# JacobPorter/FastNeighborNet

Measured on AMD Instinct MI355X. Metric: sec to circular order, n=32768 taxa (+ achieved HBM GB/s), lower is better.
Workload: dtype f64

## Files before the change

fastneighbornet_amd/csrc/fnn_hip.hip:

```cpp
#include <hip/hip_runtime.h>

#include <dlfcn.h>

#include <cmath>
#include <new>

#include "fnn_chain.h"
#include "fnn_engine.h"

namespace fnn {

struct fnn_nccl_id { char internal[FNN_COMM_ID_BYTES]; };

constexpr int SCAN_TW = 512;
constexpr int SCAN_TH = 32;
constexpr int SCAN_THREADS = 256;

static_assert(sizeof(Cand) == 24, "rec_publish / rec_fetch move a Cand as three 8-byte words");
__device__ inline uint64_t rec_check_word(const Cand& c, uint32_t tag) {
    return __builtin_bit_cast(uint64_t, c.q) ^ (c.key * 0x9E3779B97F4A7C15ULL) ^
           ((uint64_t)(uint32_t)c.si | ((uint64_t)(uint32_t)c.sj << 32)) ^ (((uint64_t)tag + 1ULL) * 0xBF58476D1CE4E5B9ULL);
}
__device__ inline void rec_publish(Cand* p, const Cand& c, uint64_t* chk, uint32_t tag) {
    __hip_atomic_store(chk, rec_check_word(c, tag), __ATOMIC_RELAXED, __HIP_MEMORY_SCOPE_AGENT);
    uint64_t* w = (uint64_t*)p;
    __hip_atomic_store(w + 0, __builtin_bit_cast(uint64_t, c.q), __ATOMIC_RELAXED, __HIP_MEMORY_SCOPE_AGENT);
    __hip_atomic_store(w + 1, c.key, __ATOMIC_RELAXED, __HIP_MEMORY_SCOPE_AGENT);
    __hip_atomic_store(w + 2, (uint64_t)(uint32_t)c.si | ((uint64_t)(uint32_t)c.sj << 32), __ATOMIC_RELAXED, __HIP_MEMORY_SCOPE_AGENT);
}
__device__ inline Cand rec_fetch(const Cand* p) {
    uint64_t* w = (uint64_t*)p;
    const uint64_t a = __hip_atomic_load(w + 0, __ATOMIC_RELAXED, __HIP_MEMORY_SCOPE_AGENT);
    const uint64_t b = __hip_atomic_load(w + 1, __ATOMIC_RELAXED, __HIP_MEMORY_SCOPE_AGENT);
    const uint64_t x = __hip_atomic_load(w + 2, __ATOMIC_RELAXED, __HIP_MEMORY_SCOPE_AGENT);
    Cand c;
    c.q = __builtin_bit_cast(double, a);
    c.key = b;
// ... 665 lines not shown
    if (!d.st->done) {
        for (int i = threadIdx.x; i < nrecs; i += 1024) {
            Cand c = src[i];
            if (cand_better(c, best)) best = c;
        }
    }
    return block_reduce<16>(best, sh);
}

__global__ __launch_bounds__(1024) void k_reduce_local(Dev d, int nrecs) {
    __shared__ Cand sh[16];
    Cand best = reduce_records(d, d.recs, nrecs, sh);
    if (threadIdx.x == 0) d.gsend[0] = best;
}


template <int EPT>
struct ChainLds {
    double wtot[CH_T / 64];
    double s;
    int slot_count;
    int32_t E[CH_T];
    int32_t flags[CH_T];
    int32_t slot[CH_T];
    uint64_t own[CH_T], sc[CH_T];
    double vals[CH_NSLOT][EPT];
    double spv[CH_T];
    ChRec prec[CH_NSLOT];
    double pend_A0[CH_NSLOT];
    int32_t pend_cnt[CH_NSLOT];
    uint64_t wk[CH_T / 64];
    int32_t wr[CH_T / 64];
    int32_t fail;
};

__device__ __forceinline__ uint64_t shfl_up_u64(uint64_t v, int d) {
    return (uint64_t)__shfl_up((unsigned long long)v, d, 64);
}
__device__ __forceinline__ int readlane_i32(int v, int lane) { return __builtin_amdgcn_readlane(v, lane); }
__device__ __forceinline__ uint64_t readlane_u64(uint64_t v, int lane) {
    uint32_t lo = (uint32_t)__builtin_amdgcn_readlane((int)(uint32_t)v, lane);
    uint32_t hi = (uint32_t)__builtin_amdgcn_readlane((int)(uint32_t)(v >> 32), lane);
    return ((uint64_t)hi << 32) | lo;
}

__device__ __forceinline__ uint64_t readfirstlane_u64(uint64_t v) {
    uint32_t lo = (uint32_t)__builtin_amdgcn_readfirstlane((int)(uint32_t)v);
    uint32_t hi = (uint32_t)__builtin_amdgcn_readfirstlane((int)(uint32_t)(v >> 32));
    return ((uint64_t)hi << 32) | lo;
}

__device__ __forceinline__ void chain_serial_global(double& s, const double* buf, int start, int cnt, int m) {
    for (int i = 0; i < cnt; i++)
        if (start + i < m) s += buf[chain_addr(start + i)];
}

__device__ int g_chain_form = 2;
__device__ int g_chain_stop_after = 0;

template <int EPT, int MODE = 0>
__device__ __forceinline__ double block_chain_sum(const double* __restrict__ buf, int m, int guard_bits, ChainLds<EPT>& L,
                                  ChainStats* stats) {
    const int stop_after = stats ? g_chain_stop_after : 0;
    static_assert(EPT % 2 == 0 && EPT <= 64, "EPT");
    const int tid = threadIdx.x, lane = tid & 63, w = tid >> 6;
    ChainStats cs{0, 0, 0, 0};
    if (tid == 0) L.s = 0.0;
    for (int base = 0; base < m; base += CH_T * EPT) {
        double s_in = 0.0;
        if (MODE != 2) {
        if (tid == 0) L.slot_count = 0;
        static_assert(EPT == CH_EPT, "the buffer layout is fixed to CH_EPT addends per thread");
        double a[EPT];
        const int idx0 = base + tid * EPT;
        const double* src = buf + base + 2 * tid;
#pragma unroll
        for (int i = 0; i < EPT; i += 2) {
            double2 v = make_double2(0.0, 0.0);
            if (idx0 + i < m) v = *reinterpret_cast<const double2*>(src + (i >> 1) * (2 * CH_T));
            a[i] = v.x;
            a[i + 1] = (idx0 + i + 1 < m) ? v.y : 0.0;
        }
        double loc = 0.0;
#pragma unroll
        for (int i = 0; i < EPT; i++) loc += a[i];
        double inc = loc;
#pragma unroll
        for (int d = 1; d < 64; d <<= 1) {
            const double t = __shfl_up(inc, d, 64);
            if (lane >= d) inc += t;
        }
// ... 155 lines not shown
        if (!tm) { r.kind = CHR_CONST; r.E0 = E_first; r.c0 = mono_inc_bits(msum(ci, inm)); return r; }
        const int jt = __builtin_ctzll(tm);
        const unsigned long long lo = inm & ((1ULL << jt) - 1ULL), hi = inm & ~((2ULL << jt) - 1ULL);
        r.kind = CHR_SPLIT; r.E0 = E_first; r.E1 = E_first;
        r.c0 = mono_inc_bits(msum(ci, lo)); r.c1 = mono_inc_bits(msum(ci, hi));
        r.sp = __builtin_bit_cast(double, readlane_u64(f2u(al), jt));
        return r;
    }
    const int js = __builtin_ctzll(bad);
    const unsigned long long lo = inm & ((1ULL << js) - 1ULL), hi = inm & ~((2ULL << js) - 1ULL);
    int32_t E1 = -1;
    if (hi) {
        const int jn = __builtin_ctzll(hi);
        E1 = __builtin_amdgcn_readlane(El, jn);
        if (__ballot(((hi >> lane) & 1ULL) && (!okl || El != E1))) return r;
    }
    bool tie0 = false, inv0 = false, tie1 = false, inv1 = false;
    const double c0l = lo ? konst(E_first, tie0, inv0) : 0.0;
    const double c1l = hi ? konst(E1, tie1, inv1) : 0.0;
    if (__ballot((((lo >> lane) & 1ULL) && (tie0 || inv0)) || (((hi >> lane) & 1ULL) && (tie1 || inv1)))) return r;
    r.kind = CHR_SPLIT;
    r.E0 = lo ? E_first : -1; r.c0 = lo ? mono_inc_bits(msum(c0l, lo)) : 0;
    r.E1 = hi ? E1 : -1; r.c1 = hi ? mono_inc_bits(msum(c1l, hi)) : 0;
    r.sp = __builtin_bit_cast(double, readlane_u64(f2u(al), js));
    return r;
}

template <int EPT>
__device__ __attribute__((noinline)) double block_chain_sum_rare(const double* __restrict__ buf, int m, int guard_bits, ChainLds<EPT>* L,
                                                               ChainStats* stats) {
    return block_chain_sum<EPT>(buf, m, guard_bits, *L, stats);
}

template <int EPT>
__device__ __forceinline__ double block_chain_sum2(const double* __restrict__ buf, int m, int guard_bits, ChainLds<EPT>& L,
                                                   ChainStats* stats) {
    static_assert(EPT == CH_EPT, "the buffer layout is fixed to CH_EPT addends per thread");
    const int tid = threadIdx.x, lane = tid & 63, w = tid >> 6;
    ChainStats cs{0, 0, 0, 0};
    if (tid == 0) { L.s = 0.0; L.fail = 0; }
    for (int base = 0; base < m; base += CH_T * EPT) {
        if (tid == 0) L.slot_count = 0;
        double a[EPT];
        const int idx0 = base + tid * EPT;
        const double* src = buf + base + 2 * tid;
#pragma unroll
        for (int i = 0; i < EPT; i += 2) {
            double2 v = make_double2(0.0, 0.0);
            if (idx0 + i < m) v = *reinterpret_cast<const double2*>(src + (i >> 1) * (2 * CH_T));
            a[i] = v.x;
            a[i + 1] = (idx0 + i + 1 < m) ? v.y : 0.0;
        }
        double l4[4] = {0.0, 0.0, 0.0, 0.0};
#pragma unroll
        for (int i = 0; i < EPT; i++) l4[i & 3] += a[i];
        const double loc = (l4[0] + l4[1]) + (l4[2] + l4[3]);
        double inc = loc;
#pragma unroll
        for (int d = 1; d < 64; d <<= 1) {
            const double t = __shfl_up(inc, d, 64);
            if (lane >= d) inc += t;
        }
        if (lane == 63) L.wtot[w] = inc;
        __syncthreads();
        double wpre = 0.0;
        for (int k = 0; k < w; k++) wpre += L.wtot[k];
        const double s_in = L.s;
        const double A0 = s_in + (wpre + (inc - loc));
        const int cnt = idx0 >= m ? 0 : (m - idx0 < EPT ? m - idx0 : EPT);
        ChRec r;
        r.kind = CHR_EMPTY; r.E0 = r.E1 = -1; r.c0 = r.c1 = 0; r.sp = 0.0;
        int slot = -1;
        if (cnt > 0) {
            int32_t E = -1;
            int nt = 0;
            uint64_t c = 0;
            if (chain_predict(A0, A0 + loc, guard_bits != 0, E) && chain_consts(a, 0, cnt, E, c, &nt, nullptr) && nt == 0) {
                r.kind = CHR_CONST; r.E0 = E; r.c0 = c;
            } else {
                r.kind = CHR_SERIAL;
                slot = atomicAdd(&L.slot_count, 1);
                if (slot < CH_NSLOT) {
#pragma unroll
                    for (int i = 0; i < EPT; i++) L.vals[slot][i] = a[i];
                    L.pend_A0[slot] = A0;
                    L.pend_cnt[slot] = cnt;
                } else slot = -1;
            }
        }
        __syncthreads();
        {
            const int ns = L.slot_count < CH_NSLOT ? L.slot_count : CH_NSLOT;
            for (int sl = w; sl < ns; sl += CH_T / 64) {
                const double al = lane < EPT ? L.vals[sl][lane < EPT ? lane : 0] : 0.0;
                const ChRec pr = chain_record_wave(al, L.pend_cnt[sl], L.pend_A0[sl], guard_bits != 0);
                if (lane == 0) L.prec[sl] = pr;
            }
        }
        __syncthreads();
        if (slot >= 0) r = L.prec[slot];
        const int32_t tailE = r.kind == CHR_CONST ? r.E0 : (r.kind == CHR_SPLIT ? r.E1 : -2);
        int32_t prevTail = __shfl_up(tailE, 1, 64);
        L.E[tid] = tailE;
        __syncthreads();
        if (lane == 0) prevTail = tid > 0 ? L.E[tid - 1] : -2;
        const bool ebreak = r.kind == CHR_CONST && prevTail != r.E0;
        int rr = (r.kind == CHR_SPLIT || r.kind == CHR_SERIAL || ebreak) ? 1 : 0;
        uint64_t kk = r.kind == CHR_CONST ? r.c0 : (r.kind == CHR_SPLIT ? (r.E1 >= 0 ? r.c1 : 0) : 0);
        const int r_own = rr;
        const uint64_t k_own = kk;
#pragma unroll
        for (int d = 1; d < 64; d <<= 1) {
            const int pr = __shfl_up(rr, d, 64);
            const uint64_t pk = shfl_up_u64(kk, d);
            if (lane >= d) {
                if (!rr) { const uint64_t t = pk + kk; kk = t > (1ULL << 60) ? (1ULL << 60) : t; }
                rr |= pr;
            }
        }
        if (lane == 63) { L.wr[w] = rr; L.wk[w] = kk; }
        __syncthreads();
        uint64_t X = 0;
        for (int q = 0; q < w; q++) { const uint64_t t = X + L.wk[q]; X = L.wr[q] ? L.wk[q] : (t > (1ULL << 60) ? (1ULL << 60) : t); }
        uint64_t after;
        { const uint64_t t = X + kk; after = rr ? kk : (t > (1ULL << 60) ? (1ULL << 60) : t); }
        uint64_t xin = shfl_up_u64(after, 1);
        if (lane == 0) xin = X;
        (void)r_own; (void)k_own;
        const bool evt = r.kind == CHR_SPLIT || r.kind == CHR_SERIAL || (ebreak && xin != 0);
        __syncthreads();
        L.E[tid] = prevTail;
        L.flags[tid] = r.kind | (evt ? 4 : 0);
        L.slot[tid] = r.kind == CHR_SERIAL ? slot : r.E0;
        L.own[tid] = r.c0;
        L.sc[tid] = xin;
        L.spv[tid] = r.sp;
        const int lastT = ((m - base < CH_T * EPT ? m - base : CH_T * EPT) - 1) / EPT;
        if (tid == lastT) { L.wk[0] = after; L.wr[0] = tailE; }
        __syncthreads();
        if (r.kind == CHR_SERIAL && tid <= lastT) cs.mixed++;
        if (w == 0) {
            uint64_t sb = readfirstlane_u64(f2u(s_in));
            bool ok = true;
            auto apply = [&](int E, uint64_t c) {
                if (c == 0) return;
                if (mono_apply_pattern(sb, E, c, c)) cs.runs++;
                else ok = false;
            };
            for (int ww = 0; ww < CH_T / 64 && ok; ww++) {
                if (ww * 64 > lastT) break;
                const int id = ww * 64 + lane;
                const int rf = L.flags[id], rEin = L.E[id], rs = L.slot[id];
                const uint64_t rc0 = L.own[id], rx = L.sc[id];
                const double rsp = L.spv[id];
                unsigned long long em = __ballot((rf & 4) != 0 && id <= lastT);
                while (em && ok) {
                    const int e = __builtin_ctzll(em);
                    em &= em - 1;
                    const int kind = readlane_i32(rf, e) & 3, Ein = readlane_i32(rEin, e), sl = readlane_i32(rs, e);
                    const uint64_t x = readlane_u64(rx, e), c0 = readlane_u64(rc0, e);
                    if (kind == CHR_CONST) apply(Ein, x);
                    else if (kind == CHR_SPLIT) {
                        const int E0 = sl;
                        if (E0 >= 0 && E0 == Ein) { const uint64_t t = x + c0; apply(E0, t > (1ULL << 60) ? (1ULL << 60) : t); }
                        else { apply(Ein, x); if (E0 >= 0) apply(E0, c0); }
                        if (!ok) break;
                        const double sv = u2f(sb) + u2f(readlane_u64(f2u(rsp), e));
                        sb = readfirstlane_u64(f2u(sv));
                    } else {
                        apply(Ein, x);
                        if (!ok) break;
                        double sv = u2f(sb);
                        if (sl >= 0) {
                            const double* pv = L.vals[sl];
#pragma unroll
                            for (int j = 0; j < EPT; j++) sv += pv[j];
                        } else chain_serial_global(sv, buf, base + (ww * 64 + e) * EPT, EPT, m);
                        sb = readfirstlane_u64(f2u(sv));
                    }
                }
            }
            if (ok) apply((int)L.wr[0], L.wk[0]);
            if (lane == 0) { L.s = u2f(sb); if (!ok) L.fail = 1; }
        }
        __syncthreads();
        if (L.fail) break;
    }
    __syncthreads();
    if (L.fail) {
        ChainStats c1{0, 0, 0, 0};
        const double r1 = block_chain_sum_rare<EPT>(buf, m, guard_bits, &L, stats ? &c1 : nullptr);
        if (stats && tid == 0) { stats->runs = cs.runs + c1.runs; stats->mixed = cs.mixed + c1.mixed; stats->run_fail = 1 + c1.run_fail; stats->thread_fail = c1.thread_fail; }
        return r1;
    }
    if (stats) {
        __shared__ int mixed_total;
        if (tid == 0) mixed_total = 0;
        __syncthreads();
        if (cs.mixed) atomicAdd(&mixed_total, cs.mixed);
        __syncthreads();
        if (tid == 0) { cs.mixed = mixed_total; *stats = cs; }
    }
    return L.s;
}

struct PreSrc { const double *pD, *pSx, *pT; int64_t pld; };
__device__ __forceinline__ void build_targets_wave(State& st, const Dev& d, const PreSrc& src, const int32_t pendU, const int32_t tpU, const double* tfin) {
    const int lane = threadIdx.x & 63;
    const int nops = __builtin_amdgcn_readfirstlane(st.nops);
    const int U = __builtin_amdgcn_readfirstlane(st.U), m = __builtin_amdgcn_readfirstlane(st.m);
    const int ev_finish = __builtin_amdgcn_readfirstlane(st.ev_finish);
    static_assert(sizeof(Op) == 32, "Op is read as 8 dwords");
    const int opw = lane < 8 * MAX_OPS ? reinterpret_cast<const int32_t*>(st.ops)[lane] : 0;
    int err = 0;
    int Sl = -1, nS = 0;
    auto add_slot = [&](int sl) {
        if (__ballot(lane < nS && Sl == sl)) return;
        if (nS >= MAX_S) { err = 5; return; }
        if (lane == nS) Sl = sl;
        nS++;
    };
// ... 764 lines not shown
        return;
    }
    if (st->stall || st->la_hit) {
        if (HELP && threadIdx.x == 0) job_post(d, jobtag, 0u);
        return;
    }
    state_in(S.lst, st);
    if (threadIdx.x == 0) S.tkon = 0;
    Cand best = reduce_records(d, src, st->rl_active ? 1 : nrecs, shc);
    __syncthreads();
    decide_step<HELP, false>(d, S, L, best, jobtag);
    __syncthreads();
    if (threadIdx.x == 0) S.lst.rl_active = 0;
    __syncthreads();
    state_out(st, S.lst);
}

constexpr int TRK_THREADS = 1024;
constexpr int TRK_GROUP = 16;
constexpr int TRK_FLAG = 32 * 65;
constexpr int TRK_BAD = 32 * 67;

__device__ __forceinline__ void chain_workgroup(const Dev& d, ChainLds<CH_EPT>& L) {
    State* st = d.st;
    if (!st->chain_pending) return;
    const int32_t cU = st->chain_U, cm = st->chain_m;
    const unsigned evtag = (unsigned)st->n_events;
    const double usx = block_chain_sum2<CH_EPT>(d.chain, cm, CH_GUARD_BITS, L, nullptr);
    if (threadIdx.x == 0) {
        __hip_atomic_store(reinterpret_cast<uint64_t*>(d.Sx + cU), __builtin_bit_cast(uint64_t, usx), __ATOMIC_RELAXED, __HIP_MEMORY_SCOPE_AGENT);
        __hip_atomic_store(reinterpret_cast<uint64_t*>(d.Sx + cU + 1), __builtin_bit_cast(uint64_t, usx), __ATOMIC_RELAXED, __HIP_MEMORY_SCOPE_AGENT);
        __hip_atomic_store(reinterpret_cast<uint64_t*>(&upre_behind_ticket(d)->usx), __builtin_bit_cast(uint64_t, usx), __ATOMIC_RELAXED, __HIP_MEMORY_SCOPE_AGENT);
        asm volatile("s_waitcnt vmcnt(0)" ::: "memory");
        __threadfence();
        __hip_atomic_store(d.ticket + TRK_FLAG, evtag, __ATOMIC_RELAXED, __HIP_MEMORY_SCOPE_AGENT);
    }
}

__device__ __forceinline__ void sweep_exact_item(const Dev& d, int64_t r, const TrackArgs& ta, Cand& bx) {
    const int32_t half = (ta.m + 1) / 2;
    const int32_t fi = ta.nf0 + (int32_t)(r / half), cp = (int32_t)(r % half);
    if (fi >= ta.nf) return;
    const int32_t f0 = fresh_slot(d, fi, ta.m);
    if (f0 < 0) return;
    const int32_t s2 = 2 * cp;
    if (s2 >= ta.m || s2 == f0) return;
    const double* F0 = d.D + (int64_t)f0 * d.ld + s2;
    const double* F1 = F0 + d.ld;
    const double a0 = F0[0], a1 = F0[1], b0 = F1[0], b1 = F1[1];
    if (f0 > s2)
        scan_micro(f0, s2, ta.m, ta.twoP, ta.cm2, a0, a1, b0, b1, d.Sx[f0], d.Sx[f0 + 1], d.spos[f0], d.spos[f0 + 1],
                   d.Sx[s2], d.Sx[s2 + 1], d.spos[s2], d.spos[s2 + 1], bx);
    else
        scan_micro(s2, f0, ta.m, ta.twoP, ta.cm2, a0, b0, a1, b1, d.Sx[s2], d.Sx[s2 + 1], d.spos[s2], d.spos[s2 + 1],
                   d.Sx[f0], d.Sx[f0 + 1], d.spos[f0], d.spos[f0 + 1], bx);
}

constexpr int TRK_REC_U = 1024;

struct SpecialOut { double val, tu, tv; };
__device__ __forceinline__ SpecialOut special_wave(const Dev& d, const State& lst, double* blk, double* sxl, double* tl, int32_t* berr, double* chain_dst) {
    const int lane = threadIdx.x & 63;
    const int nS = __builtin_amdgcn_readfirstlane(lst.nS);
    const int32_t Sl = lane < nS ? lst.S[lane < MAX_S ? lane : 0] : -1;
    const int m_old = __builtin_amdgcn_readfirstlane(lst.m_old), twoP_old = 2 * __builtin_amdgcn_readfirstlane(lst.P_old);
    const int m = __builtin_amdgcn_readfirstlane(lst.m), twoP = 2 * __builtin_amdgcn_readfirstlane(lst.P);
    const int xs = __builtin_amdgcn_readfirstlane(lst.xs), ys = __builtin_amdgcn_readfirstlane(lst.ys);
// ... 363 lines not shown
                    c = rec_fetch(&d.recs[TRK_REC_U + i]);
                    if (rec_check_word(c, tag) != __hip_atomic_load(d.rchk + TRK_REC_U + i, __ATOMIC_RELAXED, __HIP_MEMORY_SCOPE_AGENT)) stale = true;
                    if (cand_better(c, bu)) bu = c;
                }
            }
            stale = __ballot(stale) != 0ULL;
            if (!stale) break;
            reread = true;
            __threadfence();
        }
        b = wave_reduce(b);
        if (ta.approx) bu = wave_reduce(bu);
        if (threadIdx.x == 0) {
            sh[0] = b;
            shu[0] = bu;
            if (badword != 0u) {
                d.ticket[TRK_BAD] = 0u;
                lastflag = 2;
            }
            if (stale) lastflag = 2;
            if (reread) S.lst.n_ev_persistent++;
        }
    }
    __syncthreads();
    best = sh[0];
    bestu = shu[0];
    if (lastflag == 2) {
        giveup = true;
        if (d.strict && threadIdx.x == 0) S.lst.error = 13;
    }
    __syncthreads();
    TRK_TICK(5);
    if (ta.approx && !giveup) {
        const double dmax = __builtin_bit_cast(double, st->dmax_bits);
        const double margin = 2.0 * eps_u + 192.0 * 1.1102230246251565e-16 * ((double)st->n + 4.0) * dmax + 1e-300;
        const bool certain = (bestu.q - margin > best.q) || (bestu.q == inf_f64());
        if (!certain) {
            if (threadIdx.x == 0) {
                const unsigned want = evtag0;
                const long long t_wait = (long long)wall_clock64();
                while (__hip_atomic_load(d.ticket + TRK_FLAG, __ATOMIC_RELAXED, __HIP_MEMORY_SCOPE_AGENT) != want) {
                    if ((long long)wall_clock64() - t_wait > TRK_WAIT_TICKS) { lst.error = 10; break; }
                    __builtin_amdgcn_s_sleep(2);
                }
                __threadfence();
                lst.n_sweep_waits++;
            }
            __syncthreads();
            Cand bx;
            bx = cand_none();
            for (int64_t r = threadIdx.x; r < items - ta.np; r += TRK_THREADS) sweep_exact_item(d, r, ta, bx);
            bx = block_reduce<TRK_THREADS / 64>(bx, sh);
            if (threadIdx.x == 0) sh[0] = bx;
            __syncthreads();
            bx = sh[0];
            if (cand_better(bx, best)) best = bx;
        }
    }
    if (giveup) { best = cand_none(); }
    if (threadIdx.x == 0) {
        *d.ticket = 0u;
        lst.ev_timed = timed;
        if (giveup) lst.n_sweep_waits++;
        la_track_done(dl, best, ta);
        lst.stall = (!lst.la_hit && !has_scan) ? 1 : 0;
        if (lst.stall) lst.n_stalled++;
    }
    __syncthreads();
// ... 117 lines not shown
__global__ __launch_bounds__(CH_T) void k_chain_flush(Dev d) {
    __shared__ ChainLds<CH_EPT> L;
    chain_workgroup(d, L);
    __syncthreads();
    if (threadIdx.x == 0) d.st->chain_pending = 0;
}

constexpr int SER_CHUNK = 8192;
__device__ __forceinline__ double serial_chain_sum(const double* buf, int m, double* ser) {
    double s = 0.0;
    for (int base = 0; base < m; base += SER_CHUNK) {
        const int cnt = m - base < SER_CHUNK ? m - base : SER_CHUNK;
        for (int i = threadIdx.x; i < cnt; i += CH_T) ser[i] = buf[chain_addr(base + i)];
        __syncthreads();
        if (threadIdx.x == 0) {
#pragma unroll 8
            for (int i = 0; i < cnt; i++) s += ser[i];
        }
        __syncthreads();
    }
    return s;
}

__global__ __launch_bounds__(CH_T) void k_finalize(Dev d) {
    __shared__ ChainLds<CH_EPT> L;
    __shared__ double ser[SER_CHUNK];
    State* st = d.st;
    if (!st->ev_active || st->stall) return;
    double usx = 0.0;
    if (!st->ev_finish) usx = st->nonneg ? block_chain_sum2<CH_EPT>(d.chain, st->m, CH_GUARD_BITS, L, nullptr) : serial_chain_sum(d.chain, st->m, ser);
    if (threadIdx.x == 0) finalize(d, usx);
}

template <int EPT>
__global__ __launch_bounds__(CH_T) void k_test_chain(const double* buf, int m, int guard_bits, double* out, ChainStats* stats) {
    __shared__ ChainLds<EPT> L;
    double r = g_chain_form == 1 ? block_chain_sum<EPT>(buf, m, guard_bits, L, stats) : block_chain_sum2<EPT>(buf, m, guard_bits, L, stats);
    if (threadIdx.x == 0) *out = r;
}

__global__ __launch_bounds__(256) void k_init(Dev d) { init_thread(d, blockIdx.x * 256 + threadIdx.x); }

__global__ __launch_bounds__(256) void k_synth(Dev d, uint64_t seed, int dist) {
    int64_t c = (int64_t)blockIdx.x * 256 + threadIdx.x;
    int64_t r = blockIdx.y;
    if (c >= d.n) return;
    double v = 0.0;
    if (r < c) v = synth_entry(d.n, r, c, seed, dist);
    else if (c < r) v = synth_entry(d.n, c, r, seed, dist);
    d.D[r * d.ld + c] = v;
}

__global__ __launch_bounds__(256) void k_unpack(Dev d, const double* __restrict__ stage, int64_t p0, int32_t row0) {
    const int64_t r = row0 + (int64_t)blockIdx.y;
    const int64_t c = (int64_t)blockIdx.x * 256 + threadIdx.x;
    if (c <= r || c >= d.n) return;
    d.D[r * d.ld + c] = __builtin_nontemporal_load(stage + (packed_row_base(d.n, r) + c - p0));
}

__global__ __launch_bounds__(256) void k_mirror(Dev d) {
    __shared__ double tile[32][33];
    const int bx = blockIdx.x, by = blockIdx.y;
    if (bx < by) return;
    const int tx = threadIdx.x & 31, ty = threadIdx.x >> 5;
    for (int k = ty; k < 32; k += 8) {
        const int64_t r = (int64_t)by * 32 + k, c = (int64_t)bx * 32 + tx;
        tile[k][tx] = (r < d.n && c < d.n && r < c) ? d.D[r * d.ld + c] : 0.0;
    }
    __syncthreads();
    for (int k = ty; k < 32; k += 8) {
// ... 312 lines not shown
        if (!HIPOK(hipMemcpyAsync(&hb, d_bad, sizeof(int), hipMemcpyDeviceToHost, stream)) ||
            !HIPOK(hipStreamSynchronize(stream)))
            return FNN_EHIP;
        *bad = hb;
        return FNN_OK;
    }
    int32_t launch_prep_screen(const Dev& d, int64_t nrows) {
        const int64_t want = (nrows * d.ld + 255) / 256;
        launch(TC_OTHER, false, k_prep_screen, dim3((unsigned)(want < 8192 ? (want > 0 ? want : 1) : 8192)), dim3(256), d, nrows);
        return launched();
    }
    int32_t launch_init(const Dev& d) {
        reset_timing();
        rx_exact_seen = 0; rx_helpers = 0;
        launch(TC_OTHER, false, k_init, grid1(d.n), dim3(256), d);
        return launched();
    }

    dim3 scan_dims(const Dev& d, int32_t m_bound) const {
        int nt = (scan_tile_count(m_bound) + d.world - 1) / d.world;
        return dim3((unsigned)(nt < scan_grid ? (nt > 0 ? nt : 1) : scan_grid));
    }
    bool screen_off = false;
    bool keep_generic_screen() const { return false; }
    bool use_screen(const Dev& d, int32_t m_bound) const { return d.H != nullptr && !screen_off && m_bound >= screen_min_m; }
    int enqueue_scan(const Dev& d, int32_t m_bound, bool sched) {
        const bool screen = use_screen(d, m_bound);
        const bool tscan = timing != 0 && (sched || !screen), tall = timing == 2;
        const bool has_scan = sched || !screen || unsched_scans;
        if (d.la) {
            const bool help = rx_helpers > 0;
            const int fb = (sched || !screen) ? 1 : 0, hs = has_scan ? 1 : 0, tk = ticks ? 1 : 0;
            track_tag = (track_tag % 0x7FFFFFEu) + 1u;
            launch(TC_TRACK, tall, help ? k_track<true> : k_track<false>, dim3(track_grid + 1 + (help ? TRK_NHELP : 0)), dim3(TRK_THREADS),
                   d, fb, fb, hs, track_group, tk, track_tag);
        }
        if (screen && !has_scan) return 0;
        if (screen) {
            static constexpr decltype(&k_screen<true, true>) variants[2][2] = {{k_screen<true, true>, k_screen<false, true>},
                                                                               {k_screen<true, false>, k_screen<false, false>}};
            int nt = (tri_tile_count(m_bound, SCR_TH, SCR_R) + d.world - 1) / d.world;
            const int want = sched ? scan_grid : unsched_grid;
            launch(TC_SCREEN, tscan, variants[!sched][!scan_nt], dim3((unsigned)(nt < want ? (nt > 0 ? nt : 1) : want)), dim3(256), d);
            if (d.la) launch(TC_EMIT, tall, k_emit, dim3(emit_grid), dim3(256), d);
            launch(TC_RESOLVE, tall, k_resolve, dim3(RES_BLOCKS), dim3(1024), d);
            if (tscan) scan_launches++;
            return RES_BLOCKS;
        }
        if (relaxed_min > 0 && m_bound > relaxed_min) {
            int g = relaxed_grid > 0 ? relaxed_grid : (m_bound >= 12288 ? m_bound / 4096 : 1);
            launch(TC_OTHER, tall, k_relaxed, dim3(g > RL_GMAX ? RL_GMAX : g), dim3(RL_T), d, ticks ? 1 : 0);
        }
        const dim3 gs = scan_dims(d, m_bound);
        launch(TC_SCAN, tscan, scan_nt ? k_scan<true> : k_scan<false>, gs, dim3(SCAN_THREADS), d);
        if (tscan) plain_launches++;
        return (int)gs.x;
    }
    void enqueue_rest(const Dev& d, int32_t m_bound, const Cand* src, int nrecs) {
        const bool tall = timing == 2, help = rx_helpers > 0;
        if (nrecs > 0) {
            track_tag = (track_tag % 0x7FFFFFEu) + 1u;
            launch(TC_DECIDE, tall, help ? k_decide<true> : k_decide<false>, dim3(1 + (help ? TRK_NHELP : 0)), dim3(CH_T), d, src, nrecs, track_tag);
        }
        launch(TC_UPDATE, tall, k_update, dim3(grid1(m_bound).x + 1), dim3(256), d, defer_chain ? 1 : 0, ticks ? 1 : 0);
        if (!defer_chain) launch(TC_OTHER, tall, k_finalize, dim3(1), dim3(CH_T), d);
    }
    int32_t launch_event(const Dev& d, int32_t m_bound, bool sched) {
// ... 227 lines not shown
    return FNN_OK;
}
int32_t fnn_comm_init_rccl(fnn_handle* h, int32_t world, int32_t rank, const uint8_t* id, const char* rccl_path) {
    FNN_NEED(h);
    if (!id) return fnn::fail(FNN_EINVAL, "fnn_comm_init_rccl: id is NULL");
    FNN_TRY(
        int32_t rc = h->eng.comm_set(1, world, rank);
        if (rc != FNN_OK) return rc;
        if (h->eng.comm_mode == 0) return FNN_OK;
        rc = h->eng.be.comm_init_rccl(world, rank, id, rccl_path);
        if (rc != FNN_OK) { h->eng.comm_set(0, 1, 0); return fnn::fail(rc, h->eng.be.err()); }
        return FNN_OK;
    )
}
int32_t fnn_comm_init_host(fnn_handle* h, int32_t world, int32_t rank, fnn_allgather_fn fn, void* ctx) {
    FNN_NEED(h);
    if (world > 1 && !fn) return fnn::fail(FNN_EINVAL, "fnn_comm_init_host: callback is NULL");
    FNN_TRY(
        int32_t rc = h->eng.comm_set(2, world, rank);
        if (rc != FNN_OK) return rc;
        h->eng.host_fn = fn;
        h->eng.host_ctx = ctx;
        return FNN_OK;
    )
}

int32_t fnn_test_chain_sum(int32_t device, const double* host_buf, int32_t m, int32_t guard_bits, int32_t ept,
                           double* out, int32_t* stats4) {
    if (!host_buf || m < 0 || !out || ept != fnn::CH_EPT)
        return fnn::fail(FNN_EINVAL, "fnn_test_chain_sum: bad arguments (ept must be 32)");
    hipError_t e;
    if ((e = hipSetDevice(device)) != hipSuccess) return fnn::fail(FNN_EHIP, hipGetErrorString(e));
    const size_t cap = (size_t)fnn::round_up(m > 0 ? m : 1, fnn::CH_SC);
    std::vector<double> perm(cap, 0.0);
    for (int32_t i = 0; i < m; i++) perm[(size_t)fnn::chain_addr(i)] = host_buf[i];
    double* dbuf = nullptr; double* dout = nullptr; fnn::ChainStats* dst = nullptr;
    if (hipMalloc((void**)&dbuf, sizeof(double) * cap) != hipSuccess || hipMalloc((void**)&dout, 8) != hipSuccess ||
        hipMalloc((void**)&dst, sizeof(fnn::ChainStats)) != hipSuccess) {
        (void)hipFree(dbuf); (void)hipFree(dout); (void)hipFree(dst);
        return fnn::fail(FNN_ENOMEM, "fnn_test_chain_sum: hipMalloc failed");
    }
    (void)hipMemcpy(dbuf, perm.data(), sizeof(double) * cap, hipMemcpyHostToDevice);
    {
        int stop = 0;
        if (const char* ev = std::getenv("FNN_CHAIN_STOP")) stop = std::atoi(ev);
        (void)hipMemcpyToSymbol(HIP_SYMBOL(fnn::g_chain_stop_after), &stop, sizeof(int));
        int form = stop ? 1 : 2;
        if (const char* ev = std::getenv("FNN_CHAIN_FORM")) form = std::atoi(ev);
        (void)hipMemcpyToSymbol(HIP_SYMBOL(fnn::g_chain_form), &form, sizeof(int));
    }
    hipLaunchKernelGGL(fnn::k_test_chain<fnn::CH_EPT>, dim3(1), dim3(fnn::CH_T), 0, 0, dbuf, m, guard_bits, dout, dst);
    e = hipDeviceSynchronize();
    if (std::getenv("FNN_CHAIN_TIME")) {
        hipEvent_t e0, e1;
        (void)hipEventCreate(&e0); (void)hipEventCreate(&e1);
        (void)hipEventRecord(e0, 0);
        for (int i = 0; i < 50; i++)
            hipLaunchKernelGGL(fnn::k_test_chain<fnn::CH_EPT>, dim3(1), dim3(fnn::CH_T), 0, 0, dbuf, m, guard_bits, dout, dst);
        (void)hipEventRecord(e1, 0);
        (void)hipEventSynchronize(e1);
        float ms = 0.f;
        (void)hipEventElapsedTime(&ms, e0, e1);
        std::fprintf(stderr, "[fnn] k_test_chain m=%d: %.2f us per launch\n", m, ms * 1e3 / 50);
        (void)hipEventDestroy(e0); (void)hipEventDestroy(e1);
    }
    fnn::ChainStats hs{0, 0, 0, 0};
    if (e == hipSuccess) e = hipMemcpy(out, dout, 8, hipMemcpyDeviceToHost);
    if (e == hipSuccess) e = hipMemcpy(&hs, dst, sizeof(hs), hipMemcpyDeviceToHost);
    (void)hipFree(dbuf); (void)hipFree(dout); (void)hipFree(dst);
    if (e != hipSuccess) return fnn::fail(FNN_EHIP, std::string("fnn_test_chain_sum: ") + hipGetErrorString(e));
    if (stats4) { stats4[0] = hs.runs; stats4[1] = hs.mixed; stats4[2] = hs.run_fail; stats4[3] = hs.thread_fail; }
    return FNN_OK;
}

int32_t fnn_stream_probe(int32_t device, int64_t bytes, int32_t reps, double* gbps_out) {
    if (bytes < (1 << 20) || reps < 1 || !gbps_out) return fnn::fail(FNN_EINVAL, "fnn_stream_probe: bad arguments");
    hipError_t e;
    if ((e = hipSetDevice(device)) != hipSuccess) return fnn::fail(FNN_EHIP, hipGetErrorString(e));
    void* p = nullptr;
    double* sink = nullptr;
    if ((e = hipMalloc(&p, (size_t)bytes)) != hipSuccess) return fnn::fail(FNN_ENOMEM, hipGetErrorString(e));
    if ((e = hipMalloc((void**)&sink, 8)) != hipSuccess) { (void)hipFree(p); return fnn::fail(FNN_ENOMEM, hipGetErrorString(e)); }
    (void)hipMemset(p, 0, (size_t)bytes);
    hipEvent_t e0, e1;
    (void)hipEventCreate(&e0);
    (void)hipEventCreate(&e1);
    int64_t n16 = bytes / 16;
    dim3 g(256 * 8);
    hipLaunchKernelGGL(fnn::k_stream, g, dim3(256), 0, 0, (const double2*)p, n16, sink);
    (void)hipEventRecord(e0, 0);
    for (int i = 0; i < reps; i++) hipLaunchKernelGGL(fnn::k_stream, g, dim3(256), 0, 0, (const double2*)p, n16, sink);
    (void)hipEventRecord(e1, 0);
    e = hipEventSynchronize(e1);
    float ms = 0.f;
    (void)hipEventElapsedTime(&ms, e0, e1);
    (void)hipEventDestroy(e0);
    (void)hipEventDestroy(e1);
    (void)hipFree(p);
    (void)hipFree(sink);
    if (e != hipSuccess || ms <= 0.f) return fnn::fail(FNN_EHIP, "fnn_stream_probe: timing failed");
    *gbps_out = (double)bytes * reps / (ms * 1e-3) / 1e9;
    return FNN_OK;
}

}
```

include/fastnn.h:

```cpp
#ifndef FASTNN_H
#define FASTNN_H

#include <stdint.h>

#ifdef __cplusplus
extern "C" {
#endif

#define FASTNN_ABI_VERSION 2

typedef enum fnn_status {
    FNN_OK      = 0,
    FNN_EINVAL  = -1,
    FNN_ENOMEM  = -2,
    FNN_EHIP    = -3,
    FNN_ERCCL   = -4,
    FNN_ESTATE  = -5,
    FNN_ECAPACITY = -6,
    FNN_EINEXACT = -7
} fnn_status;

enum { FNN_KIND_2WAY = 2, FNN_KIND_3WAY = 3, FNN_KIND_4WAY = 4, FNN_KIND_FINISH = 5 };

typedef struct fnn_opts {
// ... 122 lines not shown
    int64_t outer_iterations;
    int64_t cg_calls;
    int64_t cg_iterations;
    int64_t nsplits;
    double  t_solve_s;
    int64_t reserved[3];
    int32_t route;
    int32_t certified;
    double  kkt_violation;
    double  final_threshold_rel;
    int64_t n_set_aside;
    int64_t capacity;
    int64_t free_set_peak;
    int32_t giveup_reason;
    int32_t pad_;
    int64_t entered, screened_out, departed;
    double  t_alloc_s;
    int64_t reserved2[4];
} fnn_sw_stats;
enum { FNN_SW_ROUTE_CLOSED_FORM = 0, FNN_SW_ROUTE_FROM_BELOW = 1, FNN_SW_ROUTE_REFERENCE = 2 };
enum { FNN_SW_GIVEUP_NONE = 0, FNN_SW_GIVEUP_CAPACITY = 1,
       FNN_SW_GIVEUP_STEPS = 2,
       FNN_SW_GIVEUP_NUMERIC = 3,
       FNN_SW_GIVEUP_DEPARTED = 4,
       FNN_SW_GIVEUP_SETUP = 5 };
int32_t fnn_split_weights_f64(const double* D, int32_t n, int64_t ld, const int32_t* ordering, int32_t device,
                              double* weights_out, fnn_sw_stats* stats);
int32_t fnn_split_weights_sparse_f64(const double* D, int32_t n, int64_t ld, const int32_t* ordering, int32_t device, double threshold,
                                     int64_t* index_out, double* weight_out, int64_t capacity, int64_t* count_out, fnn_sw_stats* stats);
int32_t fnn_split_weights_release_cache(void);

int32_t fnn_test_chain_sum(int32_t device, const double* host_buf, int32_t m, int32_t guard_bits,
                           int32_t ept, double* out, int32_t* stats4);

int32_t fnn_stream_probe(int32_t device, int64_t bytes, int32_t reps, double* gbps_out);

#ifdef __cplusplus
}
#endif
#endif
```

Before: 1.296.

## Rework block chain sum with DPP scans, short-input path, and fewer barriers

Replaces the shuffle-based wave prefix scans in block_chain_sum2 with DPP row/broadcast scans, and replaces the serial cross-wave loops with a wave-level scan. It adds a single-wave serial path for short inputs and skips a barrier when there are no serial slots. The event walk now visits only waves that flagged events. Separately, it drops a __threadfence after s_waitcnt in the update publish, shrinks the track grid to one block in fallback mode, reads margin fields from LDS, and adds tick profiling for the test kernel. These lower barrier and scan latency in the chain-sum hot loop. The dropped fence risks memory-ordering bugs.

```diff
diff --git a/fastneighbornet_amd/csrc/fnn_hip.hip b/fastneighbornet_amd/csrc/fnn_hip.hip
--- a/fastneighbornet_amd/csrc/fnn_hip.hip
+++ b/fastneighbornet_amd/csrc/fnn_hip.hip
@@ -3,6 +3,7 @@
 #include <dlfcn.h>
 
 #include <cmath>
+#include <limits>
 #include <new>
 
 #include "fnn_chain.h"
@@ -734,7 +735,14 @@
     uint64_t wk[CH_T / 64];
     int32_t wr[CH_T / 64];
     int32_t fail;
+    int32_t wtail[CH_T / 64], whead[CH_T / 64];
+    uint64_t emask[CH_T / 64];
+    uint64_t open_k;
+    int32_t open_E;
 };
+constexpr int32_t CH_NOHEAD = INT32_MIN;
+constexpr int CH_SHORT_M = 2048;
+static_assert(CH_SHORT_M <= 64 * CH_EPT, "the short form is one wave: one chunk per lane");
 
 __device__ __forceinline__ uint64_t shfl_up_u64(uint64_t v, int d) {
     return (uint64_t)__shfl_up((unsigned long long)v, d, 64);
@@ -757,8 +765,10 @@
         if (start + i < m) s += buf[chain_addr(start + i)];
 }
 
-__device__ int g_chain_form = 2;
+__device__ int g_chain_form = 0;
 __device__ int g_chain_stop_after = 0;
+constexpr int CH_NTICK = 7;
+__device__ long long g_chain_ticks[CH_NTICK];
 
 template <int EPT, int MODE = 0>
 __device__ __forceinline__ double block_chain_sum(const double* __restrict__ buf, int m, int guard_bits, ChainLds<EPT>& L,
@@ -980,12 +990,84 @@
     return block_chain_sum<EPT>(buf, m, guard_bits, *L, stats);
 }
 
+template <int CTRL, int ROW_MASK>
+__device__ __forceinline__ uint32_t dpp_or0(uint32_t v) {
+    return (uint32_t)__builtin_amdgcn_update_dpp(0, (int)v, CTRL, ROW_MASK, 0xf, false);
+}
+template <int CTRL, int ROW_MASK>
+__device__ __forceinline__ uint64_t dpp_or0_u64(uint64_t v) {
+    const uint32_t lo = dpp_or0<CTRL, ROW_MASK>((uint32_t)v), hi = dpp_or0<CTRL, ROW_MASK>((uint32_t)(v >> 32));
+    return ((uint64_t)hi << 32) | lo;
+}
+__device__ __forceinline__ uint32_t lane_below_u32(uint32_t v) {
+    const uint32_t inrow = dpp_or0<0x111, 0xf>(v), across = dpp_or0<0x142, 0xe>(v);
+    return (threadIdx.x & 15) ? inrow : across;
+}
+__device__ __forceinline__ uint64_t lane_below_u64(uint64_t v) {
+    return ((uint64_t)lane_below_u32((uint32_t)(v >> 32)) << 32) | lane_below_u32((uint32_t)v);
+}
+__device__ __forceinline__ uint64_t sat60(uint64_t t) { return t > (1ULL << 60) ? (1ULL << 60) : t; }
+template <bool ROWS_ONLY>
+__device__ __forceinline__ double scan_add_f64(double x) {
+#define FNN_SCAN_STEP(CTRL, MASK) x += u2f(dpp_or0_u64<CTRL, MASK>(f2u(x)))
+    FNN_SCAN_STEP(0x111, 0xf); FNN_SCAN_STEP(0x112, 0xf); FNN_SCAN_STEP(0x114, 0xf); FNN_SCAN_STEP(0x118, 0xf);
+    if (!ROWS_ONLY) { FNN_SCAN_STEP(0x142, 0xa); FNN_SCAN_STEP(0x143, 0xc); }
+#undef FNN_SCAN_STEP
+    return x;
+}
+template <bool ROWS_ONLY>
+__device__ __forceinline__ void scan_seg(int& rr, uint64_t& kk) {
+#define FNN_SCAN_STEP(CTRL, MASK) do { const int pr = (int)dpp_or0<CTRL, MASK>((uint32_t)rr); const uint64_t pk = dpp_or0_u64<CTRL, MASK>(kk); \
+        if (!rr) kk = sat60(pk + kk); rr |= pr; } while (0)
+    FNN_SCAN_STEP(0x111, 0xf); FNN_SCAN_STEP(0x112, 0xf); FNN_SCAN_STEP(0x114, 0xf); FNN_SCAN_STEP(0x118, 0xf);
+    if (!ROWS_ONLY) { FNN_SCAN_STEP(0x142, 0xa); FNN_SCAN_STEP(0x143, 0xc); }
+#undef FNN_SCAN_STEP
+}
+
 template <int EPT>
+__device__ __forceinline__ double chain_short_sum(const double* __restrict__ buf, int m, ChainLds<EPT>& L) {
+    const int tid = threadIdx.x;
+    if (tid < 64) {
+        double a[EPT];
+        const double* src = buf + 2 * tid;
+#pragma unroll
+        for (int j = 0; j < EPT / 2; j++) {
+            double2 v = make_double2(0.0, 0.0);
+            if (tid * EPT + 2 * j < m) v = *reinterpret_cast<const double2*>(src + j * (2 * CH_T));
+            a[2 * j] = v.x;
+            a[2 * j + 1] = tid * EPT + 2 * j + 1 < m ? v.y : 0.0;
+        }
+        double sv = 0.0;
+        const int nch = (m + EPT - 1) / EPT;
+        for (int t = 0; t < nch; t++) {
+            double s = u2f(readlane_u64(f2u(sv), t > 0 ? t - 1 : 0));
+            if (t == 0) s = 0.0;
+#pragma unroll
+            for (int i = 0; i < EPT; i++) s += a[i];
+            sv = s;
+        }
+        const double res = nch > 0 ? u2f(readlane_u64(f2u(sv), nch > 0 ? nch - 1 : 0)) : 0.0;
+        if (tid == 0) L.s = res;
+    }
+    __syncthreads();
+    return L.s;
+}
+
+template <int EPT, bool PROF = false>
 __device__ __forceinline__ double block_chain_sum2(const double* __restrict__ buf, int m, int guard_bits, ChainLds<EPT>& L,
-                                                   ChainStats* stats) {
+                                                   ChainStats* stats, int short_below = CH_SHORT_M) {
     static_assert(EPT == CH_EPT, "the buffer layout is fixed to CH_EPT addends per thread");
     const int tid = threadIdx.x, lane = tid & 63, w = tid >> 6;
+    const int wu = __builtin_amdgcn_readfirstlane(w);
+    if (m < short_below && m <= 64 * EPT) {
+        if (stats && tid == 0) *stats = ChainStats{0, 0, 0, 0};
+        return chain_short_sum<EPT>(buf, m, L);
+    }
     ChainStats cs{0, 0, 0, 0};
+    const bool prof = PROF && stats != nullptr && tid == 0;
+    long long tk[CH_NTICK] = {0, 0, 0, 0, 0, 0, 0};
+#define CH_TICK(k, dep) do { if (prof) { asm volatile("" :: "v"(dep) : "memory"); tk[k] = (long long)wall_clock64(); } } while (0)
+    CH_TICK(0, tid);
     if (tid == 0) { L.s = 0.0; L.fail = 0; }
     for (int base = 0; base < m; base += CH_T * EPT) {
         if (tid == 0) L.slot_count = 0;
@@ -1003,18 +1085,16 @@
 #pragma unroll
         for (int i = 0; i < EPT; i++) l4[i & 3] += a[i];
         const double loc = (l4[0] + l4[1]) + (l4[2] + l4[3]);
-        double inc = loc;
-#pragma unroll
-        for (int d = 1; d < 64; d <<= 1) {
-            const double t = __shfl_up(inc, d, 64);
-            if (lane >= d) inc += t;
-        }
+        CH_TICK(1, loc);
+        const double inc = scan_add_f64<false>(loc);
         if (lane == 63) L.wtot[w] = inc;
         __syncthreads();
-        double wpre = 0.0;
-        for (int k = 0; k < w; k++) wpre += L.wtot[k];
+        const double wsc = scan_add_f64<true>(lane < CH_T / 64 ? L.wtot[lane & (CH_T / 64 - 1)] : 0.0);
+        const double wbelow = u2f(readlane_u64(f2u(wsc), wu > 0 ? wu - 1 : 0));
+        const double wpre = wu > 0 ? wbelow : 0.0;
         const double s_in = L.s;
         const double A0 = s_in + (wpre + (inc - loc));
+        CH_TICK(2, A0);
         const int cnt = idx0 >= m ? 0 : (m - idx0 < EPT ? m - idx0 : EPT);
         ChRec r;
         r.kind = CHR_EMPTY; r.E0 = r.E1 = -1; r.c0 = r.c1 = 0; r.sp = 0.0;
@@ -1039,54 +1119,58 @@
         __syncthreads();
         {
             const int ns = L.slot_count < CH_NSLOT ? L.slot_count : CH_NSLOT;
-            for (int sl = w; sl < ns; sl += CH_T / 64) {
-                const double al = lane < EPT ? L.vals[sl][lane < EPT ? lane : 0] : 0.0;
-                const ChRec pr = chain_record_wave(al, L.pend_cnt[sl], L.pend_A0[sl], guard_bits != 0);
-                if (lane == 0) L.prec[sl] = pr;
-            }
-        }
+            if (ns > 0) {
+                for (int sl = w; sl < ns; sl += CH_T / 64) {
+                    const double al = lane < EPT ? L.vals[sl][lane < EPT ? lane : 0] : 0.0;
+                    const ChRec pr = chain_record_wave(al, L.pend_cnt[sl], L.pend_A0[sl], guard_bits != 0);
+                    if (lane == 0) L.prec[sl] = pr;
+                }
+                __syncthreads();
+                if (slot >= 0) r = L.prec[slot];
+            }
+        }
+        CH_TICK(3, r.kind);
+        const int32_t tailE = r.kind == CHR_CONST ? r.E0 : (r.kind == CHR_SPLIT ? r.E1 : -2);
+        int32_t prevTail = (int32_t)lane_below_u32((uint32_t)tailE);
+        int rr = (r.kind == CHR_SPLIT || r.kind == CHR_SERIAL || (lane != 0 && r.kind == CHR_CONST && prevTail != r.E0)) ? 1 : 0;
+        uint64_t kk = r.kind == CHR_CONST ? r.c0 : (r.kind == CHR_SPLIT ? (r.E1 >= 0 ? r.c1 : 0) : 0);
+        scan_seg<false>(rr, kk);
+        if (lane == 63) { L.wr[w] = rr; L.wk[w] = kk; L.wtail[w] = tailE; }
+        if (lane == 0) L.whead[w] = r.kind == CHR_CONST ? r.E0 : CH_NOHEAD;
         __syncthreads();
-        if (slot >= 0) r = L.prec[slot];
-        const int32_t tailE = r.kind == CHR_CONST ? r.E0 : (r.kind == CHR_SPLIT ? r.E1 : -2);
-        int32_t prevTail = __shfl_up(tailE, 1, 64);
-        L.E[tid] = tailE;
-        __syncthreads();
-        if (lane == 0) prevTail = tid > 0 ? L.E[tid - 1] : -2;
+        int sr = 0;
+        uint64_t sk = 0;
+        int32_t hq = CH_NOHEAD, tq = -2;
+        if (lane < CH_T / 64) {
+            sr = L.wr[lane]; sk = L.wk[lane]; hq = L.whead[lane];
+            if (lane > 0) tq = L.wtail[lane - 1];
+        }
+        const bool ebq = hq != CH_NOHEAD && tq != hq;
+        sr |= ebq ? 1 : 0;
+        const bool eb0 = ((__ballot(ebq) >> wu) & 1ULL) != 0ULL;
+        scan_seg<true>(sr, sk);
+        const uint64_t xbelow = readlane_u64(sk, wu > 0 ? wu - 1 : 0);
+        const uint64_t X = wu > 0 ? xbelow : 0;
+        const int32_t tbelow = readlane_i32(tq, wu);
+        if (lane == 0) prevTail = tbelow;
         const bool ebreak = r.kind == CHR_CONST && prevTail != r.E0;
-        int rr = (r.kind == CHR_SPLIT || r.kind == CHR_SERIAL || ebreak) ? 1 : 0;
-        uint64_t kk = r.kind == CHR_CONST ? r.c0 : (r.kind == CHR_SPLIT ? (r.E1 >= 0 ? r.c1 : 0) : 0);
-        const int r_own = rr;
-        const uint64_t k_own = kk;
-#pragma unroll
-        for (int d = 1; d < 64; d <<= 1) {
-            const int pr = __shfl_up(rr, d, 64);
-            const uint64_t pk = shfl_up_u64(kk, d);
-            if (lane >= d) {
-                if (!rr) { const uint64_t t = pk + kk; kk = t > (1ULL << 60) ? (1ULL << 60) : t; }
-                rr |= pr;
-            }
-        }
-        if (lane == 63) { L.wr[w] = rr; L.wk[w] = kk; }
-        __syncthreads();
-        uint64_t X = 0;
-        for (int q = 0; q < w; q++) { const uint64_t t = X + L.wk[q]; X = L.wr[q] ? L.wk[q] : (t > (1ULL << 60) ? (1ULL << 60) : t); }
-        uint64_t after;
-        { const uint64_t t = X + kk; after = rr ? kk : (t > (1ULL << 60) ? (1ULL << 60) : t); }
-        uint64_t xin = shfl_up_u64(after, 1);
+        const uint64_t after = (rr || eb0) ? kk : sat60(X + kk);
+        uint64_t xin = lane_below_u64(after);
         if (lane == 0) xin = X;
-        (void)r_own; (void)k_own;
         const bool evt = r.kind == CHR_SPLIT || r.kind == CHR_SERIAL || (ebreak && xin != 0);
-        __syncthreads();
+        const int lastT = ((m - base < CH_T * EPT ? m - base : CH_T * EPT) - 1) / EPT;
+        const unsigned long long evm = __ballot(evt && tid <= lastT);
         L.E[tid] = prevTail;
         L.flags[tid] = r.kind | (evt ? 4 : 0);
         L.slot[tid] = r.kind == CHR_SERIAL ? slot : r.E0;
         L.own[tid] = r.c0;
         L.sc[tid] = xin;
         L.spv[tid] = r.sp;
-        const int lastT = ((m - base < CH_T * EPT ? m - base : CH_T * EPT) - 1) / EPT;
-        if (tid == lastT) { L.wk[0] = after; L.wr[0] = tailE; }
+        if (lane == 0) L.emask[w] = evm;
+        if (tid == lastT) { L.open_k = after; L.open_E = tailE; }
         __syncthreads();
         if (r.kind == CHR_SERIAL && tid <= lastT) cs.mixed++;
+        CH_TICK(4, tid);
         if (w == 0) {
             uint64_t sb = readfirstlane_u64(f2u(s_in));
             bool ok = true;
@@ -1095,13 +1179,16 @@
                 if (mono_apply_pattern(sb, E, c, c)) cs.runs++;
                 else ok = false;
             };
-            for (int ww = 0; ww < CH_T / 64 && ok; ww++) {
-                if (ww * 64 > lastT) break;
+            const uint64_t gm = lane < CH_T / 64 ? L.emask[lane & (CH_T / 64 - 1)] : 0ULL;
+            unsigned long long groups = __ballot(gm != 0ULL);
+            while (groups && ok) {
+                const int ww = __builtin_ctzll(groups);
+                groups &= groups - 1;
+                unsigned long long em = readlane_u64(gm, ww);
                 const int id = ww * 64 + lane;
                 const int rf = L.flags[id], rEin = L.E[id], rs = L.slot[id];
                 const uint64_t rc0 = L.own[id], rx = L.sc[id];
                 const double rsp = L.spv[id];
-                unsigned long long em = __ballot((rf & 4) != 0 && id <= lastT);
                 while (em && ok) {
                     const int e = __builtin_ctzll(em);
                     em &= em - 1;
@@ -1110,7 +1197,7 @@
                     if (kind == CHR_CONST) apply(Ein, x);
                     else if (kind == CHR_SPLIT) {
                         const int E0 = sl;
-                        if (E0 >= 0 && E0 == Ein) { const uint64_t t = x + c0; apply(E0, t > (1ULL << 60) ? (1ULL << 60) : t); }
+                        if (E0 >= 0 && E0 == Ein) apply(E0, sat60(x + c0));
                         else { apply(Ein, x); if (E0 >= 0) apply(E0, c0); }
                         if (!ok) break;
                         const double sv = u2f(sb) + u2f(readlane_u64(f2u(rsp), e));
@@ -1128,13 +1215,18 @@
                     }
                 }
             }
-            if (ok) apply((int)L.wr[0], L.wk[0]);
+            if (ok) apply((int)L.open_E, L.open_k);
             if (lane == 0) { L.s = u2f(sb); if (!ok) L.fail = 1; }
         }
         __syncthreads();
+        CH_TICK(5, tid);
         if (L.fail) break;
     }
     __syncthreads();
+    CH_TICK(6, tid);
+    if (prof)
+        for (int k = 0; k < CH_NTICK; k++) g_chain_ticks[k] = tk[k];
+#undef CH_TICK
     if (L.fail) {
         ChainStats c1{0, 0, 0, 0};
         const double r1 = block_chain_sum_rare<EPT>(buf, m, guard_bits, &L, stats ? &c1 : nullptr);
@@ -1965,7 +2057,6 @@
         __hip_atomic_store(reinterpret_cast<uint64_t*>(d.Sx + cU + 1), __builtin_bit_cast(uint64_t, usx), __ATOMIC_RELAXED, __HIP_MEMORY_SCOPE_AGENT);
         __hip_atomic_store(reinterpret_cast<uint64_t*>(&upre_behind_ticket(d)->usx), __builtin_bit_cast(uint64_t, usx), __ATOMIC_RELAXED, __HIP_MEMORY_SCOPE_AGENT);
         asm volatile("s_waitcnt vmcnt(0)" ::: "memory");
-        __threadfence();
         __hip_atomic_store(d.ticket + TRK_FLAG, evtag, __ATOMIC_RELAXED, __HIP_MEMORY_SCOPE_AGENT);
     }
 }
@@ -2395,8 +2486,8 @@
     __syncthreads();
     TRK_TICK(5);
     if (ta.approx && !giveup) {
-        const double dmax = __builtin_bit_cast(double, st->dmax_bits);
-        const double margin = 2.0 * eps_u + 192.0 * 1.1102230246251565e-16 * ((double)st->n + 4.0) * dmax + 1e-300;
+        const double dmax = __builtin_bit_cast(double, lst.dmax_bits);
+        const double margin = 2.0 * eps_u + 192.0 * 1.1102230246251565e-16 * ((double)lst.n + 4.0) * dmax + 1e-300;
         const bool certain = (bestu.q - margin > best.q) || (bestu.q == inf_f64());
         if (!certain) {
             if (threadIdx.x == 0) {
@@ -2580,10 +2671,11 @@
     if (threadIdx.x == 0) finalize(d, usx);
 }
 
-template <int EPT>
+template <int EPT, bool PROF>
 __global__ __launch_bounds__(CH_T) void k_test_chain(const double* buf, int m, int guard_bits, double* out, ChainStats* stats) {
     __shared__ ChainLds<EPT> L;
-    double r = g_chain_form == 1 ? block_chain_sum<EPT>(buf, m, guard_bits, L, stats) : block_chain_sum2<EPT>(buf, m, guard_bits, L, stats);
+    const int short_below = g_chain_form == 2 ? 0 : (g_chain_form == 3 ? 64 * EPT + 1 : CH_SHORT_M);
+    double r = g_chain_form == 1 ? block_chain_sum<EPT>(buf, m, guard_bits, L, stats) : block_chain_sum2<EPT, PROF>(buf, m, guard_bits, L, stats, short_below);
     if (threadIdx.x == 0) *out = r;
 }
 
@@ -2962,7 +3054,8 @@
             const bool help = rx_helpers > 0;
             const int fb = (sched || !screen) ? 1 : 0, hs = has_scan ? 1 : 0, tk = ticks ? 1 : 0;
             track_tag = (track_tag % 0x7FFFFFEu) + 1u;
-            launch(TC_TRACK, tall, help ? k_track<true> : k_track<false>, dim3(track_grid + 1 + (help ? TRK_NHELP : 0)), dim3(TRK_THREADS),
+            const int tgrid = fb ? 1 : track_grid;
+            launch(TC_TRACK, tall, help ? k_track<true> : k_track<false>, dim3(tgrid + 1 + (help ? TRK_NHELP : 0)), dim3(TRK_THREADS),
                    d, fb, fb, hs, track_group, tk, track_tag);
         }
         if (screen && !has_scan) return 0;
@@ -3256,7 +3349,7 @@
     hipError_t e;
     if ((e = hipSetDevice(device)) != hipSuccess) return fnn::fail(FNN_EHIP, hipGetErrorString(e));
     const size_t cap = (size_t)fnn::round_up(m > 0 ? m : 1, fnn::CH_SC);
-    std::vector<double> perm(cap, 0.0);
+    std::vector<double> perm(cap, std::numeric_limits<double>::quiet_NaN());
     for (int32_t i = 0; i < m; i++) perm[(size_t)fnn::chain_addr(i)] = host_buf[i];
     double* dbuf = nullptr; double* dout = nullptr; fnn::ChainStats* dst = nullptr;
     if (hipMalloc((void**)&dbuf, sizeof(double) * cap) != hipSuccess || hipMalloc((void**)&dout, 8) != hipSuccess ||
@@ -3269,23 +3362,34 @@
         int stop = 0;
         if (const char* ev = std::getenv("FNN_CHAIN_STOP")) stop = std::atoi(ev);
         (void)hipMemcpyToSymbol(HIP_SYMBOL(fnn::g_chain_stop_after), &stop, sizeof(int));
-        int form = stop ? 1 : 2;
+        int form = stop ? 1 : 0;
         if (const char* ev = std::getenv("FNN_CHAIN_FORM")) form = std::atoi(ev);
         (void)hipMemcpyToSymbol(HIP_SYMBOL(fnn::g_chain_form), &form, sizeof(int));
-    }
-    hipLaunchKernelGGL(fnn::k_test_chain<fnn::CH_EPT>, dim3(1), dim3(fnn::CH_T), 0, 0, dbuf, m, guard_bits, dout, dst);
+        const long long zero[fnn::CH_NTICK] = {0};
+        (void)hipMemcpyToSymbol(HIP_SYMBOL(fnn::g_chain_ticks), zero, sizeof(zero));
+    }
+    hipLaunchKernelGGL((fnn::k_test_chain<fnn::CH_EPT, false>), dim3(1), dim3(fnn::CH_T), 0, 0, dbuf, m, guard_bits, dout, dst);
     e = hipDeviceSynchronize();
     if (std::getenv("FNN_CHAIN_TIME")) {
         hipEvent_t e0, e1;
         (void)hipEventCreate(&e0); (void)hipEventCreate(&e1);
         (void)hipEventRecord(e0, 0);
         for (int i = 0; i < 50; i++)
-            hipLaunchKernelGGL(fnn::k_test_chain<fnn::CH_EPT>, dim3(1), dim3(fnn::CH_T), 0, 0, dbuf, m, guard_bits, dout, dst);
+            hipLaunchKernelGGL((fnn::k_test_chain<fnn::CH_EPT, false>), dim3(1), dim3(fnn::CH_T), 0, 0, dbuf, m, guard_bits, dout, dst);
         (void)hipEventRecord(e1, 0);
         (void)hipEventSynchronize(e1);
         float ms = 0.f;
         (void)hipEventElapsedTime(&ms, e0, e1);
         std::fprintf(stderr, "[fnn] k_test_chain m=%d: %.2f us per launch\n", m, ms * 1e3 / 50);
+        hipLaunchKernelGGL((fnn::k_test_chain<fnn::CH_EPT, true>), dim3(1), dim3(fnn::CH_T), 0, 0, dbuf, m, guard_bits, dout, dst);
+        (void)hipDeviceSynchronize();
+        long long tk[fnn::CH_NTICK] = {0};
+        if (hipMemcpyFromSymbol(tk, HIP_SYMBOL(fnn::g_chain_ticks), sizeof(tk)) == hipSuccess && tk[fnn::CH_NTICK - 1] > tk[0]) {
+            static const char* const name[fnn::CH_NTICK - 1] = {"loads", "prefix", "records", "segscan", "walk", "tail"};
+            std::fprintf(stderr, "[fnn] k_test_chain m=%d phases (us):", m);
+            for (int k = 0; k + 1 < fnn::CH_NTICK; k++) std::fprintf(stderr, " %s %.2f", name[k], (double)(tk[k + 1] - tk[k]) * 1e-2);
+            std::fprintf(stderr, "\n");
+        }
         (void)hipEventDestroy(e0); (void)hipEventDestroy(e1);
     }
     fnn::ChainStats hs{0, 0, 0, 0};
@@ -3296,6 +3400,8 @@
     if (stats4) { stats4[0] = hs.runs; stats4[1] = hs.mixed; stats4[2] = hs.run_fail; stats4[3] = hs.thread_fail; }
     return FNN_OK;
 }
+
+int32_t fnn_test_chain_short_below(void) { return fnn::CH_SHORT_M; }
 
 int32_t fnn_stream_probe(int32_t device, int64_t bytes, int32_t reps, double* gbps_out) {
     if (bytes < (1 << 20) || reps < 1 || !gbps_out) return fnn::fail(FNN_EINVAL, "fnn_stream_probe: bad arguments");
diff --git a/include/fastnn.h b/include/fastnn.h
--- a/include/fastnn.h
+++ b/include/fastnn.h
@@ -178,6 +178,7 @@
 
 int32_t fnn_test_chain_sum(int32_t device, const double* host_buf, int32_t m, int32_t guard_bits,
                            int32_t ept, double* out, int32_t* stats4);
+int32_t fnn_test_chain_short_below(void);
 
 int32_t fnn_stream_probe(int32_t device, int64_t bytes, int32_t reps, double* gbps_out);
 
```

Result: faster. 1.272, median of 6 (-1.8%).
